# team-ergo-unipi/ergo_uvo

Hardware: AMD Instinct MI355X
Metric: stereo frame-pairs/sec (detect+match+pose) @1920x1080, 3k kpts (higher is better)
Workload: dtype f32+f64

## Files before the change

### ergo_uvo_amd/csrc/surf.hip

```cpp
#include "uvo_ctx.h"
#include <type_traits>
#include <string.h>
#include "uvo_math.h"
#include <algorithm>
#include <utility>
#include <vector>
#include <string>

namespace uvo {

struct ImgPair { const uint8_t* img[2]; int32_t* sum[2]; int32_t* planes[2]; int pw, pstride; int* cand_n; int* big_n; int* surv_n; };
struct AreaTab;
struct CandOut { uvo_keypoint* cand[2]; int* count; int cap; };
struct SurvOut { Survivor* list; int* count; int cap; };
static_assert(sizeof(Survivor) == 128, "a survivor record is 32 words");
struct SortArgs { const uvo_keypoint* cand[2]; const int* cand_n; uvo_keypoint* out[2]; int* out_n[2]; int* rank; int cap;
                  int4* big_par; int* big_n; int* gate_nqa; int gate_min_features; };
struct DescArgs { const uint8_t* img[2]; uvo_keypoint* kps[2]; float* desc[2]; const int* n[2]; const float* DW;
                  const int4* big_par; const int* big_n; const int* big_large; int cap;
                  const AreaTab* tabs; const int* iscale;
                  int extended;
                  const int32_t* sum[2]; const float* ori_w; int* ori_drop; };
struct LaneArgs { ImgPair ip; int32_t* part; SurvOut sv; CandOut out; SortArgs sa; DescArgs da; uint8_t* patch; const int4* big_in; int4* big_out; int* big_large; };
static const int kStripRows = 8;
// ... 1126 lines not shown

__host__ __device__ __forceinline__ AreaTab area_tab(int dx, int ssize, double scale)
{
    AreaTab t;
    double fsx1 = dx * scale;
    double fsx2 = fsx1 + scale;
    double cellWidth = scale < ssize - fsx1 ? scale : ssize - fsx1;
    int sx1 = cv_ceil_d(fsx1), sx2 = cv_floor_d(fsx2);
    sx2 = sx2 < ssize - 1 ? sx2 : ssize - 1;
    sx1 = sx1 < sx2 ? sx1 : sx2;
    t.sx1 = sx1; t.sx2 = sx2;
    t.has_first = sx1 - fsx1 > 1e-3;
    t.a_first = (float)((sx1 - fsx1) / cellWidth);
    t.a_mid = (float)(1.0 / cellWidth);
    t.has_last = fsx2 - sx2 > 1e-3;
    double a = fsx2 - sx2; if (a > 1.) a = 1.; if (a > cellWidth) a = cellWidth;
    t.a_last = (float)(a / cellWidth);
    return t;
}

__device__ __forceinline__ uint8_t sat_u8(float v) { int iv = cv_round_f(v); return (uint8_t)(iv < 0 ? 0 : iv > 255 ? 255 : iv); }


__device__ __forceinline__ void describe_tail(const DescArgs& a, int im, int k, const int (*PATCH)[21])
{
    const int tid = threadIdx.x;
    __shared__ float DX[20][20], DY[20][20];
    __shared__ float vec[128];
    __shared__ float s_scale;
    const int dsize = a.extended ? 128 : 64;
    for (int o = tid; o < 400; o += 256) {
        int i = o / 20, j = o - i * 20;
        float dw = a.DW[o];
        float vx = (PATCH[i][j+1] - PATCH[i][j] + PATCH[i+1][j+1] - PATCH[i+1][j]) * dw;
        float vy = (PATCH[i+1][j] - PATCH[i][j] + PATCH[i+1][j+1] - PATCH[i][j+1]) * dw;
        DX[i][j] = vx; DY[i][j] = vy;
    }
    __syncthreads();
    if (tid < dsize) {
        float acc = 0.f;
        if (!a.extended) {
            int cell = tid >> 2, comp = tid & 3, ci = cell >> 2, cj = cell & 3;
            for (int y = ci * 5; y < ci * 5 + 5; y++)
                for (int x = cj * 5; x < cj * 5 + 5; x++) {
                    float t = (comp & 1) ? DY[y][x] : DX[y][x];
                    acc += (comp & 2) ? (float)fabs(t) : t;
                }
        } else {
            int cell = tid >> 3, comp = tid & 7, ci = cell >> 2, cj = cell & 3;
            for (int y = ci * 5; y < ci * 5 + 5; y++)
                for (int x = cj * 5; x < cj * 5 + 5; x++) {
                    const float tx = DX[y][x], ty = DY[y][x];
                    const float val = comp < 4 ? tx : ty, sel = comp < 4 ? ty : tx;
                    const bool take = (comp & 2) ? sel < 0 : sel >= 0;
                    if (take) acc += (comp & 1) ? (float)fabs(val) : val;
                }
        }
        vec[tid] = acc;
    }
    __syncthreads();
    if (tid == 0) {
        double square_mag = 0;
        for (int kk = 0; kk < dsize; kk++) square_mag += vec[kk] * vec[kk];
        s_scale = (float)(1. / (sqrt(square_mag) + FLT_EPSILON));
    }
    __syncthreads();
    if (tid < dsize) a.desc[im][(size_t)k * dsize + tid] = vec[tid] * s_scale;
}

static const int kTapBatch = 16;
static const int kPatchStride = 448;
__device__ __forceinline__ int sgpr_i(int v) { return __builtin_amdgcn_readfirstlane(v); }
__device__ __forceinline__ int ssel_lt(int a, int b, int x, int y)
{
    int r;
    asm volatile("s_cmp_lt_i32 %1, %2\n\ts_cselect_b32 %0, %3, %4" : "=s"(r) : "s"(a), "s"(b), "s"(x), "s"(y) : "scc");
    return r;
}
__device__ __forceinline__ float sgpr_f(float v) { return __int_as_float(__builtin_amdgcn_readfirstlane(__float_as_int(v))); }

struct ColTask { int y0, n, h1, w; float a_first, a_mid, a_last; };

template <int PX> __device__ __forceinline__ unsigned px_load(ImgRsrc rs, int voff, int soff);
template <> __device__ __forceinline__ unsigned px_load<1>(ImgRsrc rs, int voff, int soff) { return __builtin_amdgcn_raw_buffer_load_b8(rs, voff, soff, 0); }
template <> __device__ __forceinline__ unsigned px_load<2>(ImgRsrc rs, int voff, int soff) { return __builtin_amdgcn_raw_buffer_load_b16(rs, voff, soff, 0); }
template <> __device__ __forceinline__ unsigned px_load<4>(ImgRsrc rs, int voff, int soff) { return __builtin_amdgcn_raw_buffer_load_b32(rs, voff, soff, 0); }

template <int PX, int Q>
struct AreaCol {
    ImgRsrc rs; int w, h1;
    int x[Q], voff[Q];
    float acc[Q][PX];
    __device__ __forceinline__ AreaCol(ImgRsrc rs_, int w_, int h_, int lane, int xa) : rs(rs_), w(w_), h1(h_ - 1)
    {
#pragma unroll
        for (int q = 0; q < Q; q++) { x[q] = xa + PX * (lane + 64 * q); voff[q] = x[q] < w - PX ? x[q] : w - PX; }
    }
    __device__ __forceinline__ void load(const ColTask& t, int tap, unsigned (&v)[Q]) const
    {
        int y = t.y0 - tap; y = y > 0 ? y : 0; y = y < h1 ? y : h1;
        const int soff = y * w;
#pragma unroll
        for (int q = 0; q < Q; q++) v[q] = px_load<PX>(rs, voff[q], soff);
    }
    static __device__ __forceinline__ float px_times(unsigned v, int p, float alpha) { return (float)(int)((v >> (8 * p)) & 255u) * alpha; }
    __device__ __forceinline__ void first(const unsigned (&v)[Q], float alpha)
    {
#pragma unroll
        for (int q = 0; q < Q; q++)
#pragma unroll
            for (int p = 0; p < PX; p++) acc[q][p] = px_times(v[q], p, alpha);
    }
    __device__ __forceinline__ void accum(const unsigned (&v)[Q], float alpha)
    {
#pragma unroll
        for (int q = 0; q < Q; q++)
#pragma unroll
            for (int p = 0; p < PX; p++) acc[q][p] += px_times(v[q], p, alpha);
    }
    template <int N> __device__ __forceinline__ void taps_static(const ColTask& t)
    {
        unsigned v[N][Q];
#pragma unroll
        for (int i = 0; i < N; i++) load(t, i, v[i]);
        first(v[0], t.a_first);
#pragma unroll
        for (int i = 1; i < N - 1; i++) accum(v[i], t.a_mid);
        if (N > 1) accum(v[N - 1], t.a_last);
    }
    __device__ __forceinline__ void taps_any(const ColTask& t)
    {
        constexpr int B = Q == 1 ? 8 : (Q == 2 ? 7 : 4);
        const int last = t.n - 1;
        unsigned v0[Q], vl[Q], v[B][Q];
        load(t, 0, v0);
        load(t, last > 0 ? last : 0, vl);
        first(v0, t.n > 0 ? t.a_first : 0.f);
        for (int tap = 1; tap < last; tap += B) {
#pragma unroll
            for (int i = 0; i < B; i++) load(t, tap + i < last ? tap + i : last, v[i]);
#pragma unroll
            for (int i = 0; i < B; i++) accum(v[i], tap + i < last ? t.a_mid : 0.f);
        }
        accum(vl, last > 0 ? t.a_last : 0.f);
    }
    __device__ __forceinline__ void taps(const ColTask& t)
    {
        if (Q == 1) {
            switch (t.n) {
            case 1: taps_static<1>(t); break;   case 2: taps_static<2>(t); break;   case 3: taps_static<3>(t); break;
            case 4: taps_static<4>(t); break;   case 5: taps_static<5>(t); break;   case 6: taps_static<6>(t); break;
            case 7: taps_static<7>(t); break;   case 8: taps_static<8>(t); break;   case 9: taps_static<9>(t); break;
            case 10: taps_static<10>(t); break; case 11: taps_static<11>(t); break; case 12: taps_static<12>(t); break;
            case 13: taps_static<13>(t); break; case 14: taps_static<14>(t); break;
            default: taps_any(t); break;
            }
        } else if (Q == 2 && PX == 1) {
            switch (t.n) {
            case 1: taps_static<1>(t); break;   case 2: taps_static<2>(t); break;   case 3: taps_static<3>(t); break;
            case 4: taps_static<4>(t); break;   case 5: taps_static<5>(t); break;   case 6: taps_static<6>(t); break;
            case 7: taps_static<7>(t); break;   case 8: taps_static<8>(t); break;
            default: taps_any(t); break;
            }
        } else taps_any(t);
    }
    __device__ __forceinline__ void store(int lane, int start_x, int win_size, float* __restrict__ row) const
    {
        const int xlo = start_x > 0 ? start_x : 0, xhi = start_x + win_size < w ? start_x + win_size : w;
        const int sh = start_x & 3;
        float* dst = row + sh - start_x;
#pragma unroll
        for (int q = 0; q < Q; q++) {
            if (x[q] < xhi) {
                if (PX == 4) *reinterpret_cast<float4*>(dst + x[q]) = make_float4(acc[q][0], acc[q][1], acc[q][2], acc[q][3]);
                else if (PX == 2) *reinterpret_cast<float2*>(dst + x[q]) = make_float2(acc[q][0], acc[q][1]);
                else dst[x[q]] = acc[q][0];
            }
        }
        const int ilo = xlo - start_x, ihi = xhi - start_x;
        if (ilo > 0) { const float b = row[sh + ilo]; for (int i = lane; i < ilo; i += 64) row[sh + i] = b; }
        if (ihi < win_size) { const float b = row[sh + ihi - 1]; for (int i = ihi + lane; i < win_size; i += 64) row[sh + i] = b; }
    }
};

template <int PX, int Q>
__device__ __forceinline__ void area_column(ImgRsrc rs, int lane, int start_x, int win_size, const ColTask& t, float* __restrict__ row)
{
    const int xlo = start_x > 0 ? start_x : 0;
    AreaCol<PX, Q> c(rs, t.w, t.h1 + 1, lane, xlo & ~(PX - 1));
    c.taps(t);
    c.store(lane, start_x, win_size, row);
}
__device__ __forceinline__ ColTask col_task(const AreaTab& ty, int dx, int start_y, int w, int h)
{
    const int sx1 = __builtin_amdgcn_readlane(ty.sx1, dx), sx2 = __builtin_amdgcn_readlane(ty.sx2, dx);
    const float a_first = __int_as_float(__builtin_amdgcn_readlane(__float_as_int(ty.a_first), dx));
    const float a_mid = __int_as_float(__builtin_amdgcn_readlane(__float_as_int(ty.a_mid), dx));
    const float a_last = __int_as_float(__builtin_amdgcn_readlane(__float_as_int(ty.a_last), dx));
    const bool has_first = __builtin_amdgcn_readlane((int)ty.has_first, dx) != 0, has_last = __builtin_amdgcn_readlane((int)ty.has_last, dx) != 0;
    const int c_begin = has_first ? sx1 - 1 : sx1, c_end = has_last ? sx2 + 1 : sx2;
    const int bf = sgpr_i(__float_as_int(a_first)), bm = sgpr_i(__float_as_int(a_mid)), bl = sgpr_i(__float_as_int(a_last));
    ColTask t;
    t.y0 = start_y - c_begin; t.n = c_end - c_begin; t.h1 = h - 1; t.w = w;
    t.a_first = __int_as_float(ssel_lt(c_begin, sx1, bf, ssel_lt(c_begin, sx2, bm, bl)));
    t.a_mid = a_mid;
    t.a_last = __int_as_float(ssel_lt(c_end - 1, sx1, bf, ssel_lt(c_end - 1, sx2, bm, bl)));
    return t;
}

__device__ __forceinline__ void describe_keypoint(const DescArgs& a, int w, int h, int k, int im)
{
    const int tid = threadIdx.x;
    const uvo_keypoint kp = a.kps[im][k];
    const float size = kp.size;
    const float s = size * 1.2f / 9.0f;
    const int win_size = (int)((20 + 1) * s);
    if (win_size > kSmallWin) return;
    extern __shared__ __align__(16) unsigned char smem_desc[];
    float* buf = reinterpret_cast<float*>(smem_desc);
    const int bp = (win_size + 3) | 1;
    __shared__ AreaTab tab[21];
    __shared__ int PATCH[21][21];
    const uint8_t* __restrict__ img = a.img[im];
    const float win_offset = -(float)(win_size - 1) / 2;
    const int start_x = cv_round_f(kp.x + win_offset);
    const int start_y = cv_round_f(kp.y - win_offset);
    const double inv_scale = (double)21 / win_size;
    const double scale = 1. / inv_scale;
    const int iscale = cv_round_d(scale);
    const bool area_fast = fabs(scale - iscale) < DBL_EPSILON;

    if (area_fast) {
        for (int o = tid; o < 441; o += 256) {
            int dy = o / 21, dx = o - dy * 21;
            int sum = 0;
            for (int sx = 0; sx < iscale; sx++) {
                int y = start_y - (dx * iscale + sx); y = y > 0 ? y : 0; y = y < h - 1 ? y : h - 1;
                for (int sy = 0; sy < iscale; sy++) {
                    int x = start_x + dy * iscale + sy; x = x > 0 ? x : 0; x = x < w - 1 ? x : w - 1;
                    sum += img[(size_t)y * w + x];
                }
            }
            int result;
            if (iscale == 2) result = (sum + 2) >> 2;
            else { float sc = 1.f / (iscale * iscale); result = sat_u8(sum * sc); }
            PATCH[dy][dx] = result;
        }
    } else {
        if (tid < 21) tab[tid] = area_tab(tid, win_size, scale);
        __syncthreads();
        {
            const int wv = sgpr_i(tid >> 6), lane = tid & 63;
            const AreaTab ty = tab[lane % 21];
            const int xlo = start_x > 0 ? start_x : 0, xhi = start_x + win_size < w ? start_x + win_size : w;
            const ImgRsrc rs = img_rsrc(img, w * h);
            const int sx = sgpr_i(start_x), sy = sgpr_i(start_y), ws = sgpr_i(win_size);
            if (xhi <= xlo) { for (int it = tid; it < 21 * bp; it += 256) buf[it] = 0.f; }
            else if (xhi - xlo <= 64) {
                AreaCol<1, 1> c(rs, w, h, lane, xlo);
                for (int dx = wv; dx < 21; dx += 4) { const ColTask ct = col_task(ty, dx, sy, w, h); c.taps(ct); c.store(lane, sx, ws, buf + dx * bp); }
            } else {
                AreaCol<1, 2> c(rs, w, h, lane, xlo);
                for (int dx = wv; dx < 21; dx += 4) { const ColTask ct = col_task(ty, dx, sy, w, h); c.taps(ct); c.store(lane, sx, ws, buf + dx * bp); }
            }
        }
        __syncthreads();
        for (int o = tid; o < 441; o += 256) {
            int dy = o / 21, dx = o - dy * 21;
            const AreaTab ty = tab[dy];
            const float* col = buf + dx * bp + (start_x & 3);
            float sum = 0.f;
            if (ty.has_first) sum += ty.a_first * col[ty.sx1 - 1];
            for (int r = ty.sx1; r < ty.sx2; r++) sum += ty.a_mid * col[r];
            if (ty.has_last) sum += ty.a_last * col[ty.sx2];
            PATCH[dy][dx] = sat_u8(sum);
        }
    }
    __syncthreads();
    describe_tail(a, im, k, PATCH);
}

static const int kOriRadius = 6, kOriWin = 60, kOriInc = 5, kOriSamples = 113;
__device__ __forceinline__ float fast_atan2_deg(float y, float x)
{
    const float sc = (float)(180 / 3.14159265358979323846);
    const float p1 = 0.9997878412794807f * sc, p3 = -0.3258083974640975f * sc, p5 = 0.1555786518463281f * sc, p7 = -0.04432655554792128f * sc;
    const float ax = fabsf(x), ay = fabsf(y);
    float a, c, c2;
    if (ax >= ay) { c = ay / (ax + (float)DBL_EPSILON); c2 = c * c; a = (((p7 * c2 + p5) * c2 + p3) * c2 + p1) * c; }
    else { c = ax / (ay + (float)DBL_EPSILON); c2 = c * c; a = 90.f - (((p7 * c2 + p5) * c2 + p3) * c2 + p1) * c; }
    if (x < 0) a = 180.f - a;
    if (y < 0) a = 360.f - a;
    return a;
}
__device__ __forceinline__ void ori_gradients(const int32_t* __restrict__ p, int sw, int gws, float* vx, float* vy)
{
    const float ratio = (float)gws / 4;
    const int c0 = cv_round_f(ratio * 0), c2 = cv_round_f(ratio * 2), c4 = cv_round_f(ratio * 4);
    auto box = [&](int x1, int y1, int x2, int y2) { return p[y1 * sw + x1] + p[y2 * sw + x2] - p[y2 * sw + x1] - p[y1 * sw + x2]; };
    {
        const float w0 = -1 / ((float)(c2 - c0) * (c4 - c0)), w1 = 1 / ((float)(c4 - c2) * (c4 - c0));
        double d = 0;
        d += box(c0, c0, c2, c4) * w0; d += box(c2, c0, c4, c4) * w1;
        *vx = (float)d;
    }
    {
        const float w0 = 1 / ((float)(c4 - c0) * (c2 - c0)), w1 = -1 / ((float)(c4 - c0) * (c4 - c2));
        double d = 0;
        d += box(c0, c0, c4, c2) * w0; d += box(c0, c2, c4, c4) * w1;
        *vy = (float)d;
    }
}

__global__ __launch_bounds__(256) void k_surf_orientation(DescArgs a, int w, int h)
{
    const int im = blockIdx.y, lane = threadIdx.x & 63, wv = threadIdx.x >> 6;
    const int n = *a.n[im];
    const int k = blockIdx.x * 4 + wv;
    __shared__ float sX[4][128], sY[4][128]; __shared__ int sA[4][128];
    if (k >= n) return;
    uvo_keypoint kp = a.kps[im][k];
    const float s = kp.size * 1.2f / 9.0f;
    const int gws = 2 * cv_round_f(2 * s);
    const int sum_rows = h + 1, sw = w + 1;
    const int32_t* __restrict__ sum = a.sum[im];
    int cnt_before = 0;
    for (int pass = 0; pass < 3; pass++) {
        const int cell = pass * 64 + lane;
        bool inside = false, valid = false; float vx = 0, vy = 0;
        if (cell < 169) {
            const int i = cell / 13 - kOriRadius, j = cell % 13 - kOriRadius;
            inside = i * i + j * j <= kOriRadius * kOriRadius;
            if (inside) {
                const int x = cv_round_f(kp.x + i * s - (float)(gws - 1) / 2), y = cv_round_f(kp.y + j * s - (float)(gws - 1) / 2);
                if (!(y < 0 || y >= sum_rows - gws || x < 0 || x >= sw - gws)) {
                    valid = true;
                    ori_gradients(sum + (size_t)y * sw + x, sw, gws, &vx, &vy);
                    const float wgt = a.ori_w[(i + kOriRadius) * 13 + (j + kOriRadius)];
                    vx *= wgt; vy *= wgt;
                }
            }
        }
        const unsigned long long m = __ballot(valid);
        if (valid) {
            const int pos = cnt_before + __popcll(m & ((1ull << lane) - 1ull));
            sX[wv][pos] = vx; sY[wv][pos] = vy; sA[wv][pos] = cv_round_f(fast_atan2_deg(vy, vx));
        }
        cnt_before += __popcll(m);
    }
    const int nangle = cnt_before;
    __builtin_amdgcn_fence(__ATOMIC_ACQ_REL, "wavefront");
    __builtin_amdgcn_wave_barrier();
    if (nangle == 0) { if (lane == 0) atomicAdd(a.ori_drop, 1); return; }
    float best_mod = 0.f, bx = 0.f, by = 0.f; int best_i = 1 << 30;
    for (int d = lane; d < 360 / kOriInc; d += 64) {
        const int i = d * kOriInc;
        float sumx = 0.f, sumy = 0.f;
        for (int j = 0; j < nangle; j++) {
            const int dd = abs(sA[wv][j] - i);
            if (dd < kOriWin / 2 || dd > 360 - kOriWin / 2) { sumx += sX[wv][j]; sumy += sY[wv][j]; }
        }
        const float mod = sumx * sumx + sumy * sumy;
// ... 185 lines not shown
                                        const float alpha = j < tx.sx1 ? tx.a_first : (j < tx.sx2 ? tx.a_mid : tx.a_last);
                                        b += v * alpha;
                                    }
                                    if (j + 1 >= c_end) {
                                        buf[dx][tid] = b; b = 0.f; dx++;
                                        if (dx < 21) tx = tab[dx];
                                        continue;
                                    }
                                    break;
                                }
                            }
                        }
                    }
                } else {
                    for (int e = tid; e < 21 * nr; e += 256) {
                        const int dx = e / nr, il = e - dx * nr;
                        int x = start_x + r0 + il; x = x > 0 ? x : 0; x = x < ncols1 ? x : ncols1;
                        const int c_begin = tap_begin(dx), c_end = tap_end(dx);
                        const AreaTab tx = tab[dx];
                        float b = 0.f;
                        int isum = 0;
                        for (int c0 = c_begin; c0 < c_end; c0 += 8) {
                            int v[8];
#pragma unroll
                            for (int q = 0; q < 8; q++) {
                                int y = start_y - (c0 + q); y = y > 0 ? y : 0; y = y < nrows1 ? y : nrows1;
                                v[q] = img[(size_t)y * w + x];
                            }
#pragma unroll
                            for (int q = 0; q < 8; q++) {
                                const int cc = c0 + q;
                                if (cc >= c_end) continue;
                                if (iscale) isum += v[q];
                                else {
                                    const float alpha = cc < tx.sx1 ? tx.a_first : (cc < tx.sx2 ? tx.a_mid : tx.a_last);
                                    b += v[q] * alpha;
                                }
                            }
                        }
                        if (iscale) reinterpret_cast<int*>(&buf[dx][0])[il] = isum;
                        else buf[dx][il] = b;
                    }
                }
                __syncthreads();
                if (tid < 21) {
                    if (iscale) { for (int r = 0; r < nr; r++) visum += reinterpret_cast<const int*>(&buf[tid][0])[r]; }
                    else for (int r = 0; r < nr; r++) {
                        const int rr = r0 + r;
                        const float beta = rr < ty.sx1 ? ty.a_first : (rr < ty.sx2 ? ty.a_mid : ty.a_last);
                        vsum += beta * buf[tid][r];
                    }
                }
                __syncthreads();
            }
            if (tid < 21) {
                int result;
                if (!iscale) result = sat_u8(vsum);
                else if (iscale == 2) result = (visum + 2) >> 2;
                else { const float sc = 1.f / (iscale * iscale); result = sat_u8(visum * sc); }
                patch[((size_t)im * a.cap + k) * kPatchStride + dy * 21 + tid] = (uint8_t)result;
            }
        }
        __syncthreads();
    }
}
__global__ __launch_bounds__(256) void k_descriptor_wide_finish(DescArgs a, const uint8_t* __restrict__ patch)
{
    const int im = blockIdx.y, tid = threadIdx.x;
    const int n = *a.n[im];
    __shared__ int PATCH[21][21];
    for (int k = blockIdx.x; k < n; k += gridDim.x) {
        const float s = a.kps[im][k].size * 1.2f / 9.0f;
        if ((int)((20 + 1) * s) <= kMaxWin) continue;
        const uint8_t* src = patch + ((size_t)im * a.cap + k) * kPatchStride;
        for (int o = tid; o < 441; o += 256) PATCH[o / 21][o % 21] = src[o];
        __syncthreads();
        describe_tail(a, im, k, PATCH);
        __syncthreads();
    }
}

__device__ __forceinline__ void descriptor64_small(const DescArgs& a, int w, int h, int bx, int nbx, int im)
{
    const int n = *a.n[im];
    for (int k = bx; k < n; k += nbx) {
        describe_keypoint(a, w, h, k, im);
        __syncthreads();
    }
}
static const int kBigRow = 768;
__device__ __forceinline__ void descriptor64_big(const DescArgs& a, int w, int h, uint8_t* __restrict__ patch, int bx, int nbx, int im)
{
    const int lane = threadIdx.x & 63, wv = sgpr_i(threadIdx.x >> 6);
    const int nb = a.big_n[im], nl = min(a.big_large[im], nb);
    extern __shared__ __align__(16) unsigned char smem_desc[];
    float* bufrow0 = reinterpret_cast<float*>(smem_desc) + wv * kBigRow;
    const uint8_t* __restrict__ img = a.img[im];
    const ImgRsrc rs = img_rsrc(img, w * h);
    const int nt1 = nl * 21, ntask = nt1 + (nb - nl) * 7, NW = nbx * 4, wid = bx * 4 + wv;
    auto task_of = [&](int r) { return r * NW + ((r & 1) ? NW - 1 - wid : wid); };
    auto entry_of = [&](int t) { return t < nt1 ? t / 21 : nl + (t - nt1) / 7; };
    const int tl = lane % 21;
    int4 par_next = make_int4(0, 0, 0, 0);
    AreaTab tab_next = a.tabs[tl];
    if (task_of(0) < ntask) { par_next = a.big_par[im * a.cap + entry_of(task_of(0))]; tab_next = a.tabs[min(par_next.y & 0xFFFF, kMaxWin) * 21 + tl]; }
    for (int r = 0; r * NW < ntask; r++) {
        const int t = task_of(r);
        const int4 par = par_next;
        const AreaTab ty = tab_next;
        if (task_of(r + 1) < ntask) {
            par_next = a.big_par[im * a.cap + entry_of(task_of(r + 1))];
            tab_next = a.tabs[min(par_next.y & 0xFFFF, kMaxWin) * 21 + tl];
        }
        if (t >= ntask) continue;
        const int e = entry_of(t);
        const int ncols = t < nt1 ? 1 : 3, dx0 = t < nt1 ? t - e * 21 : 3 * ((t - nt1) - (e - nl) * 7);
        const int bstride = 256;
        const int win_size = sgpr_i(par.y) & 0xFFFF, start_x = sgpr_i(par.z), start_y = sgpr_i(par.w);
        const int iscale = sgpr_i(par.y) >> 16;
        const bool area_fast = iscale != 0;
        uint8_t* out = patch + ((size_t)im * a.cap + e) * kPatchStride;
        const int xlo = start_x > 0 ? start_x : 0, xhi = start_x + win_size < w ? start_x + win_size : w;
        const bool vec_ok = (w & 3) == 0 && xlo < xhi;
        const int xa = xlo & ~3, ilo = xlo - start_x, ihi = xhi - start_x;
        if (area_fast) {
            for (int d = 0; d < ncols; d++) {
                const int dx = dx0 + d;
                int* colsum = reinterpret_cast<int*>(bufrow0 + d * bstride);
                if (vec_ok) {
                    for (int x4 = xa + 4 * lane; x4 < xhi; x4 += 256) {
                        int s0 = 0, s1 = 0, s2 = 0, s3 = 0;
                        for (int sx = 0; sx < iscale; sx++) {
                            int y = start_y - (dx * iscale + sx); y = y > 0 ? y : 0; y = y < h - 1 ? y : h - 1;
                            const unsigned v = *reinterpret_cast<const unsigned*>(img + ((unsigned)(y * w) + (unsigned)x4));
                            s0 += v & 255u; s1 += (v >> 8) & 255u; s2 += (v >> 16) & 255u; s3 += v >> 24;
                        }
                        const int c = x4 - start_x;
                        if (c >= ilo) colsum[c] = s0;
                        if (c + 1 >= ilo && c + 1 < ihi) colsum[c + 1] = s1;
                        if (c + 2 >= ilo && c + 2 < ihi) colsum[c + 2] = s2;
                        if (c + 3 >= ilo && c + 3 < ihi) colsum[c + 3] = s3;
                    }
                    if (ilo > 0) { const int v = colsum[ilo]; for (int c = lane; c < ilo; c += 64) colsum[c] = v; }
                    if (ihi < win_size) { const int v = colsum[ihi - 1]; for (int c = ihi + lane; c < win_size; c += 64) colsum[c] = v; }
                } else
                for (int c = lane; c < win_size; c += 64) {
                    int x = start_x + c; x = x > 0 ? x : 0; x = x < w - 1 ? x : w - 1;
                    int sum = 0;
                    for (int sx = 0; sx < iscale; sx++) {
                        int y = start_y - (dx * iscale + sx); y = y > 0 ? y : 0; y = y < h - 1 ? y : h - 1;
                        sum += img[(size_t)y * w + x];
                    }
                    colsum[c] = sum;
                }
            }
            __builtin_amdgcn_wave_barrier();
            if (lane < 21 * ncols) {
                const int d = lane / 21, dy = lane - d * 21;
                const int* colsum = reinterpret_cast<const int*>(bufrow0 + d * bstride);
                int sum = 0;
                for (int sy = 0; sy < iscale; sy++) sum += colsum[dy * iscale + sy];
                int result;
                if (iscale == 2) result = (sum + 2) >> 2;
                else { float sc = 1.f / (iscale * iscale); result = sat_u8(sum * sc); }
                out[dy * 21 + dx0 + d] = (uint8_t)result;
            }
        } else {
            for (int d = 0; d < ncols; d++) {
                const int dx = dx0 + d;
                float* bufrow = bufrow0 + d * bstride;
                if (vec_ok) {
// ... 259 lines not shown
            c->d_hess_order_cap = (size_t)ngroups;
        }
        UVO_HIP_TRY(c, hipMemcpyAsync(c->d_hess_order, c->h_hess_order.data(), sizeof(uint32_t) * (size_t)ngroups, hipMemcpyHostToDevice, c->stream));
        UVO_HIP_TRY(c, hipStreamSynchronize(c->stream));
        c->hess_order_key[0] = nb0; c->hess_order_key[1] = nb1; c->hess_order_key[2] = nb23;
    }
    return UVO_OK;
}

static uvo_status surf_detect_general(Ctx* c, const LaneArgs& LA, int nimg, float thr)
{
    const int w = c->img_w, h = c->img_h;
    const int no = c->p.SURF_OCTAVES_NUMBER, nl = c->p.SURF_OCTAVES_LAYERS;
    const GenLayer* tab = static_cast<const GenLayer*>(c->d_gen_tab);
    const int gx = std::min(1024, (w * h + 255) / 256);
    {
        StageTimer t(c, ST_HESSIAN_O0);
        hipLaunchKernelGGL(k_scale_space_det, dim3(gx, no * (nl + 2), nimg), dim3(256), 0, c->stream, LA, tab, c->d_gen_planes, c->gen_img_floats, w);
        UVO_HIP_TRY(c, hipGetLastError());
    }
    {
        StageTimer t(c, ST_HESSIAN_O0 + 1);
        hipLaunchKernelGGL(k_scale_space_nms, dim3(gx, no * nl, nimg), dim3(256), 0, c->stream, LA, tab, c->d_gen_planes, c->gen_img_floats, nl, w, h, thr);
        UVO_HIP_TRY(c, hipGetLastError());
    }
    return UVO_OK;
}

static uvo_status surf_detect_tuned(Ctx* c, const LaneArgs& LA, int nimg, float thr)
{
    constexpr int TW0 = kMergedTW0, TH0 = kMergedTH0, TW1 = kMergedTW1, TH1 = kO1TileRows;
    constexpr size_t lds0 = hessian_c_tile_lds<0, TW0, TH0>(), lds1 = hessian_c_tile_lds<1, TW1, TH1>(), lds = lds0 > lds1 ? lds0 : lds1;
    static_assert(lds <= 54600, "three blocks of the merged detection launch must fit a CU's 160 KB of LDS");
    const int w = c->img_w, h = c->img_h;
    const OctavePat* ops = reinterpret_cast<const OctavePat*>(c->h_octpat.data());
    const int total = merged_grid(ops).total;
    if (total > 0) {
        auto kern = k_hessian_nms_all<TW0, TH0>;
        static bool lds_raised[64] = {false};
        UVO_HIP_TRY(c, raise_dynamic_lds(c, kern, lds, lds_raised));
        StageTimer t(c, ST_HESSIAN_O0);
        HessDims hd;
        for (int o = 0; o < 4; o++) {
            OctDims& d = hd.o[o];
            for (int l = 0; l < 5; l++) { d.L[l].samples_i = ops[o].L[l].samples_i; d.L[l].samples_j = ops[o].L[l].samples_j; }
            d.rows = ops[o].rows; d.cols = ops[o].cols; d.octave = ops[o].octave;
            for (int l = 0; l < 3; l++) d.nms_margin[l] = ops[o].nms_margin[l];
        }
        Ctx::TraceRec* trh = (c->trace_on && c->trace_cur >= 0) ? &c->trace[c->trace_cur] : nullptr;
        if (trh) (void)hipEventRecord(trh->ev[6], c->stream);
        hipLaunchKernelGGL(kern, dim3(total, nimg), dim3(kP23Threads), lds, c->stream, LA, w, h, hd, thr, c->d_hess_order);
        if (trh) { (void)hipEventRecord(trh->ev[7], c->stream); trh->det_marked = true; }
        UVO_HIP_TRY(c, hipGetLastError());
    }
    {
        StageTimer t(c, ST_HESSIAN_O0 + c->p.SURF_OCTAVES_NUMBER - 1);
        hipLaunchKernelGGL(k_hessian_finish, dim3((c->surv_cap + kFinishPerWg - 1) / kFinishPerWg), dim3(256), 0, c->stream, LA, static_cast<const OctavePat*>(c->d_octpat), w, h);
        UVO_HIP_TRY(c, hipGetLastError());
    }
    return UVO_OK;
}

static uvo_status surf_order(Ctx* c, const LaneArgs& LA, int nimg)
{
    StageTimer t(c, ST_SORT);
    hipLaunchKernelGGL(k_order, dim3(1, nimg), dim3(kOrderThreads), 0, c->stream, LA, c->d_area_iscale);
    if (c->cap > kOrderCap) {
        const int tiles_max = ((c->cap + 255) / 256) * ((c->cap + kSortChunk - 1) / kSortChunk);
        hipLaunchKernelGGL(k_rank_partial, dim3(tiles_max < 512 ? tiles_max : 512, nimg), dim3(256), 0, c->stream, LA);
        hipLaunchKernelGGL(k_rank_scatter, dim3((c->cap + 255) / 256, nimg), dim3(256), 0, c->stream, LA);
        hipLaunchKernelGGL(k_big_sort, dim3(nimg), dim3(1024), 0, c->stream, LA, c->cap, c->d_area_iscale);
    }
    UVO_HIP_TRY(c, hipGetLastError());
    return UVO_OK;
}

static uvo_status surf_describe(Ctx* c, const LaneArgs& LA, int nimg)
{
    const int w = c->img_w, h = c->img_h;
    StageTimer t(c, ST_DESCRIPTOR);
    const bool wide = c->sh->surf_detection_path == 1 || widest_window(c, w, h) > kMaxWin;
    const int kWideGrid = 128;
    if (c->p.SURF_UPRIGHT) {
        const size_t lds_small = sizeof(float) * 21 * ((kSmallWin + 3) | 1), lds_big = sizeof(float) * 4 * kBigRow;
        const int nbig = 1024;
        const int hint = c->sh->kp_hint;
        int nsmall = hint > 0 ? ((hint + hint / 4 + 255) & ~255) : c->cap;
        nsmall = nsmall < 512 ? 512 : (nsmall > c->cap ? c->cap : nsmall);
        hipLaunchKernelGGL(k_descriptor64, dim3((nbig + nsmall) * nimg), dim3(256), lds_small > lds_big ? lds_small : lds_big, c->stream, DescLane{ { LA } }, w, h, nbig, nimg);
        hipLaunchKernelGGL(k_descriptor64_big_finish, dim3(1024, nimg), dim3(256), 0, c->stream, LA);
        if (wide) {
            hipLaunchKernelGGL(k_descriptor_wide<false>, dim3(21 * kWideGrid, nimg), dim3(256), 0, c->stream, LA.da, w, h, LA.patch);
            hipLaunchKernelGGL(k_descriptor_wide_finish, dim3(kWideGrid, nimg), dim3(256), 0, c->stream, LA.da, LA.patch);
        }
    } else {
        const DescArgs& da = LA.da;
        const size_t lds_rot = sizeof(float) * 21 * (kMaxWin + 1);
        static bool lds_raised[64] = {false};
        UVO_HIP_TRY(c, raise_dynamic_lds(c, k_descriptor_rot, lds_rot, lds_raised));
        hipLaunchKernelGGL(k_surf_orientation, dim3((c->cap + 3) / 4, nimg), dim3(256), 0, c->stream, da, w, h);
        hipLaunchKernelGGL(k_descriptor_rot, dim3(2048, nimg), dim3(256), lds_rot, c->stream, da, w, h);
        if (wide) {
            hipLaunchKernelGGL(k_descriptor_wide<true>, dim3(21 * kWideGrid, nimg), dim3(256), 0, c->stream, da, w, h, LA.patch);
            hipLaunchKernelGGL(k_descriptor_wide_finish, dim3(kWideGrid, nimg), dim3(256), 0, c->stream, da, LA.patch);
        }
    }
    UVO_HIP_TRY(c, hipGetLastError());
    return UVO_OK;
}

uvo_status surf_detect(Ctx* c, int nimg, int gate_min_features)
{
    UVO_TRY(surf_prepare(c, c->img_w, c->img_h));
    const LaneArgs LA = lane_args(c, nimg, gate_min_features);
    const float thr = (float)c->p.SURF_MIN_HESSIAN;
    UVO_TRY(surf_integral_launch(c, LA, nimg));
    UVO_TRY(general_path(c) ? surf_detect_general(c, LA, nimg, thr) : surf_detect_tuned(c, LA, nimg, thr));
    UVO_TRY(surf_order(c, LA, nimg));
    return surf_describe(c, LA, nimg);
}

uvo_status surf_hessian_layer_debug(Ctx* c, int octave, int layer, float* det, float* trace)
{
    const int w = c->img_w, h = c->img_h;
    if (octave < 0 || octave >= kGenMaxOctaves || layer < 0 || layer > c->p.SURF_OCTAVES_LAYERS + 1 || w <= 0) {
        c->err = "hessian_layer: octave 0..7, layer 0..SURF_OCTAVES_LAYERS + 1 of the context's parameters, after an image";
        return UVO_INVALID_ARG;
    }
    GenLayer op;
    make_gen_layer(octave, layer, w, h, &op);
    size_t n = (size_t)op.rows * op.cols;
    if (n == 0) return UVO_OK;
    float *d_det = nullptr, *d_tr = nullptr;
    UVO_HIP_TRY(c, hipMalloc(&d_det, sizeof(float) * n * 2));
    d_tr = d_det + n;
    UVO_HIP_TRY(c, hipMemsetAsync(d_det, 0, sizeof(float) * n * 2, c->stream));
    const LayerPat& lp = op.lp;
    if (lp.samples_i > 0) {
        dim3 g((lp.samples_j + 255) / 256, lp.samples_i);
        hipLaunchKernelGGL(k_hessian_layer_debug, g, dim3(256), 0, c->stream, c->d_sum[0], w, h, lp, op.step, op.rows, op.cols, d_det, d_tr);
    }
    UVO_HIP_TRY(c, hipMemcpyAsync(det, d_det, sizeof(float) * n, hipMemcpyDeviceToHost, c->stream));
    UVO_HIP_TRY(c, hipMemcpyAsync(trace, d_tr, sizeof(float) * n, hipMemcpyDeviceToHost, c->stream));
    UVO_HIP_TRY(c, hipStreamSynchronize(c->stream));
    (void)hipFree(d_det);
    return UVO_OK;
}

}
```

Baseline: 4101.

## Describe small SURF keypoints one per wavefront with direct separable area gathers

Rewrites the small-window upright descriptor so that each 64-lane wavefront handles one keypoint, instead of a whole 256-thread block per keypoint. Per-wave LDS replaces shared block buffers, and wave barriers replace block-wide __syncthreads. The area resampling now gathers each of the 441 patch entries directly, using dword buffer loads with byte alignment and perm-based edge clamping, templated on tap count, rather than a column-buffer pass followed by a row pass. The grid is shrunk 4x and the dynamic LDS for the small path is dropped. It risks numeric differences in summation order and fewer blocks in flight.

```diff
diff --git a/ergo_uvo_amd/csrc/surf.hip b/ergo_uvo_amd/csrc/surf.hip
--- a/ergo_uvo_amd/csrc/surf.hip
+++ b/ergo_uvo_amd/csrc/surf.hip
@@ -1232,8 +1232,6 @@
 struct ColTask { int y0, n, h1, w; float a_first, a_mid, a_last; };
 
 template <int PX> __device__ __forceinline__ unsigned px_load(ImgRsrc rs, int voff, int soff);
-template <> __device__ __forceinline__ unsigned px_load<1>(ImgRsrc rs, int voff, int soff) { return __builtin_amdgcn_raw_buffer_load_b8(rs, voff, soff, 0); }
-template <> __device__ __forceinline__ unsigned px_load<2>(ImgRsrc rs, int voff, int soff) { return __builtin_amdgcn_raw_buffer_load_b16(rs, voff, soff, 0); }
 template <> __device__ __forceinline__ unsigned px_load<4>(ImgRsrc rs, int voff, int soff) { return __builtin_amdgcn_raw_buffer_load_b32(rs, voff, soff, 0); }
 
 template <int PX, int Q>
@@ -1303,13 +1301,6 @@
             case 7: taps_static<7>(t); break;   case 8: taps_static<8>(t); break;   case 9: taps_static<9>(t); break;
             case 10: taps_static<10>(t); break; case 11: taps_static<11>(t); break; case 12: taps_static<12>(t); break;
             case 13: taps_static<13>(t); break; case 14: taps_static<14>(t); break;
-            default: taps_any(t); break;
-            }
-        } else if (Q == 2 && PX == 1) {
-            switch (t.n) {
-            case 1: taps_static<1>(t); break;   case 2: taps_static<2>(t); break;   case 3: taps_static<3>(t); break;
-            case 4: taps_static<4>(t); break;   case 5: taps_static<5>(t); break;   case 6: taps_static<6>(t); break;
-            case 7: taps_static<7>(t); break;   case 8: taps_static<8>(t); break;
             default: taps_any(t); break;
             }
         } else taps_any(t);
@@ -1358,76 +1349,177 @@
     return t;
 }
 
-__device__ __forceinline__ void describe_keypoint(const DescArgs& a, int w, int h, int k, int im)
-{
-    const int tid = threadIdx.x;
+static const int kWaveLds = kPatchStride + 128 * (int)sizeof(float);
+__device__ __forceinline__ void wave_sync() { __builtin_amdgcn_fence(__ATOMIC_ACQ_REL, "wavefront"); __builtin_amdgcn_wave_barrier(); }
+
+struct AreaRun { int begin, n; float wf, wm, wl; };
+static_assert(21 * sizeof(AreaRun) <= 128 * sizeof(float), "a wave keeps its runs where its descriptor vector goes");
+__device__ __forceinline__ AreaRun area_run(const AreaTab& t, bool unit)
+{
+    AreaRun r;
+    const int end = t.has_last ? t.sx2 + 1 : t.sx2;
+    r.begin = t.has_first ? t.sx1 - 1 : t.sx1; r.n = end - r.begin;
+    int bf = __float_as_int(t.a_first), bm = __float_as_int(t.a_mid), bl = __float_as_int(t.a_last);
+    asm volatile("" : "+v"(bf), "+v"(bm), "+v"(bl));
+    r.wf = __int_as_float(r.begin < t.sx1 ? bf : (r.begin < t.sx2 ? bm : bl));
+    r.wl = __int_as_float(end - 1 < t.sx1 ? bf : (end - 1 < t.sx2 ? bm : bl));
+    r.wm = __int_as_float(bm);
+    if (unit) r.wf = r.wm = r.wl = 1.f;
+    return r;
+}
+__device__ __forceinline__ float run_weight(const AreaRun& r, int i) { return i >= r.n ? 0.f : (i == r.n - 1 ? r.wl : (i == 0 ? r.wf : r.wm)); }
+
+template <int NT, bool CLAMP>
+struct RowFetch {
+    int xc, h1; unsigned sel_lo, sel_hi;
+    __device__ __forceinline__ RowFetch(int x0, int w, int h) : xc(x0), h1(h - 1), sel_lo(0), sel_hi(0)
+    {
+        if (CLAMP) {
+            xc = x0 < w - NT ? x0 : w - NT; xc = xc > 0 ? xc : 0;
+#pragma unroll
+            for (int i = 0; i < NT; i++) {
+                int x = x0 + i; x = x > 0 ? x : 0; x = x < w - 1 ? x : w - 1;
+                if (i < 4) sel_lo |= (unsigned)(x - xc) << (8 * i); else sel_hi |= (unsigned)(x - xc) << (8 * (i - 4));
+            }
+        }
+    }
+    __device__ __forceinline__ void load(ImgRsrc rs, int w, int y, unsigned (&d)[3]) const
+    {
+        if (CLAMP) { y = y > 0 ? y : 0; y = y < h1 ? y : h1; }
+        const int oa = (y * w + xc) & ~3;
+        d[0] = __builtin_amdgcn_raw_buffer_load_b32(rs, oa, 0, 0); d[1] = __builtin_amdgcn_raw_buffer_load_b32(rs, oa + 4, 0, 0);
+        d[2] = NT <= 5 ? 0u : __builtin_amdgcn_raw_buffer_load_b32(rs, oa + 8, 0, 0);
+    }
+    __device__ __forceinline__ void bytes(int w, int y, const unsigned (&d)[3], unsigned& lo, unsigned& hi) const
+    {
+        if (CLAMP) { y = y > 0 ? y : 0; y = y < h1 ? y : h1; }
+        const int sh = (y * w + xc) & 3;
+        lo = __builtin_amdgcn_alignbyte(d[1], d[0], sh); hi = __builtin_amdgcn_alignbyte(d[2], d[1], sh);
+        if (CLAMP) { const unsigned l = __builtin_amdgcn_perm(hi, lo, sel_lo), u = __builtin_amdgcn_perm(hi, lo, sel_hi); lo = l; hi = u; }
+    }
+};
+template <int NT, bool CLAMP>
+__device__ __forceinline__ float gather_entry(ImgRsrc rs, int w, int h, int start_x, int start_y, const AreaRun* __restrict__ tab, int dx, int dy)
+{
+    constexpr int B = NT <= 5 ? NT : 4;
+    float H[NT];
+    {
+        const AreaRun c = tab[dx];
+        const RowFetch<NT, CLAMP> f(start_x + tab[dy].begin, w, h);
+        const int y0 = start_y - c.begin;
+#pragma unroll
+        for (int t0 = 0; t0 < NT; t0 += B) {
+            unsigned d[B][3];
+#pragma unroll
+            for (int b = 0; b < B; b++) if (t0 + b < NT) f.load(rs, w, y0 - (t0 + b), d[b]);
+#pragma unroll
+            for (int b = 0; b < B; b++) {
+                const int t = t0 + b;
+                if (t >= NT) continue;
+                unsigned lo, hi;
+                f.bytes(w, y0 - t, d[b], lo, hi);
+                const float alpha = run_weight(c, t);
+#pragma unroll
+                for (int i = 0; i < NT; i++) {
+                    const float p = (float)(int)(((i < 4 ? lo : hi) >> (8 * (i & 3))) & 255u) * alpha;
+                    H[i] = t == 0 ? p : H[i] + p;
+                }
+            }
+        }
+    }
+    const AreaRun r = tab[dy];
+    float sum = 0.f;
+#pragma unroll
+    for (int i = 0; i < NT; i++) sum += run_weight(r, i) * H[i];
+    return sum;
+}
+template <int NT, bool CLAMP>
+__device__ __forceinline__ void gather_patch(ImgRsrc rs, int w, int h, int lane, int start_x, int start_y, const AreaRun* __restrict__ tab, int iscale, float sc, uint8_t* __restrict__ P)
+{
+    for (int j = 0; j < 7; j++) {
+        const int e = lane + 64 * j, ec = e < 441 ? e : 440;
+        const int dx = ec / 21, dy = ec - dx * 21;
+        const float sum = gather_entry<NT, CLAMP>(rs, w, h, start_x, start_y, tab, dx, dy);
+        int result;
+        if (iscale == 0) result = sat_u8(sum);
+        else {
+            const int isum = (int)sum;
+            if (iscale == 2) result = (isum + 2) >> 2;
+            else result = sat_u8(isum * sc);
+        }
+        if (e < 441) P[dy * 21 + dx] = (uint8_t)result;
+    }
+}
+template <bool EXT>
+__device__ __forceinline__ float cell_sum(const uint8_t* __restrict__ P, const float* __restrict__ DW, int d)
+{
+    const int cell = EXT ? d >> 3 : d >> 2, comp = EXT ? d & 7 : d & 3, ci = cell >> 2, cj = cell & 3;
+    float acc = 0.f;
+#pragma unroll 1
+    for (int yy = 0; yy < 5; yy++)
+#pragma unroll
+        for (int xx = 0; xx < 5; xx++) {
+            const int i = ci * 5 + yy, j = cj * 5 + xx;
+            const int p00 = P[i * 21 + j], p01 = P[i * 21 + j + 1], p10 = P[i * 21 + 21 + j], p11 = P[i * 21 + 21 + j + 1];
+            const float dw = DW[i * 20 + j];
+            const float tx = (p01 - p00 + p11 - p10) * dw;
+            const float ty = (p10 - p00 + p11 - p01) * dw;
+            if (!EXT) {
+                const float t = (comp & 1) ? ty : tx;
+                acc += (comp & 2) ? (float)fabs(t) : t;
+            } else {
+                const float val = comp < 4 ? tx : ty, sel = comp < 4 ? ty : tx;
+                const bool take = (comp & 2) ? sel < 0 : sel >= 0;
+                if (take) acc += (comp & 1) ? (float)fabs(val) : val;
+            }
+        }
+    return acc;
+}
+__device__ __forceinline__ void describe_keypoint(const DescArgs& a, ImgRsrc rs, int w, int h, int k, int im, int lane, unsigned char* __restrict__ lds)
+{
     const uvo_keypoint kp = a.kps[im][k];
     const float size = kp.size;
     const float s = size * 1.2f / 9.0f;
     const int win_size = (int)((20 + 1) * s);
     if (win_size > kSmallWin) return;
-    extern __shared__ __align__(16) unsigned char smem_desc[];
-    float* buf = reinterpret_cast<float*>(smem_desc);
-    const int bp = (win_size + 3) | 1;
-    __shared__ AreaTab tab[21];
-    __shared__ int PATCH[21][21];
-    const uint8_t* __restrict__ img = a.img[im];
+    uint8_t* P = lds;
+    float* vec = reinterpret_cast<float*>(lds + kPatchStride);
     const float win_offset = -(float)(win_size - 1) / 2;
-    const int start_x = cv_round_f(kp.x + win_offset);
-    const int start_y = cv_round_f(kp.y - win_offset);
-    const double inv_scale = (double)21 / win_size;
-    const double scale = 1. / inv_scale;
-    const int iscale = cv_round_d(scale);
-    const bool area_fast = fabs(scale - iscale) < DBL_EPSILON;
-
-    if (area_fast) {
-        for (int o = tid; o < 441; o += 256) {
-            int dy = o / 21, dx = o - dy * 21;
-            int sum = 0;
-            for (int sx = 0; sx < iscale; sx++) {
-                int y = start_y - (dx * iscale + sx); y = y > 0 ? y : 0; y = y < h - 1 ? y : h - 1;
-                for (int sy = 0; sy < iscale; sy++) {
-                    int x = start_x + dy * iscale + sy; x = x > 0 ? x : 0; x = x < w - 1 ? x : w - 1;
-                    sum += img[(size_t)y * w + x];
-                }
-            }
-            int result;
-            if (iscale == 2) result = (sum + 2) >> 2;
-            else { float sc = 1.f / (iscale * iscale); result = sat_u8(sum * sc); }
-            PATCH[dy][dx] = result;
+    const int start_x = sgpr_i(cv_round_f(kp.x + win_offset));
+    const int start_y = sgpr_i(cv_round_f(kp.y - win_offset));
+    const int ws = sgpr_i(win_size > 0 ? win_size : 0);
+    const int iscale = sgpr_i(a.iscale[ws]);
+    AreaRun* tab = reinterpret_cast<AreaRun*>(vec);
+    int el = lane; asm volatile("" : "+v"(el));
+    if (el < 21) tab[el] = area_run(a.tabs[ws * 21 + el], iscale != 0);
+    wave_sync();
+    const float sc = sgpr_f(1.f / (iscale * iscale));
+    const int nt = (ws + 20) / 21 + 1;
+    const bool inside = start_x >= 0 && start_x + ws <= w && start_y <= h - 1 && start_y - (ws - 1) >= 0;
+    if (inside) {
+        switch (nt) {
+        case 4: gather_patch<4, false>(rs, w, h, lane, start_x, start_y, tab, iscale, sc, P); break;
+        case 5: gather_patch<5, false>(rs, w, h, lane, start_x, start_y, tab, iscale, sc, P); break;
+        case 6: gather_patch<6, false>(rs, w, h, lane, start_x, start_y, tab, iscale, sc, P); break;
+        case 7: gather_patch<7, false>(rs, w, h, lane, start_x, start_y, tab, iscale, sc, P); break;
+        case 8: gather_patch<8, false>(rs, w, h, lane, start_x, start_y, tab, iscale, sc, P); break;
+        default: gather_patch<3, false>(rs, w, h, lane, start_x, start_y, tab, iscale, sc, P); break;
         }
     } else {
-        if (tid < 21) tab[tid] = area_tab(tid, win_size, scale);
-        __syncthreads();
-        {
-            const int wv = sgpr_i(tid >> 6), lane = tid & 63;
-            const AreaTab ty = tab[lane % 21];
-            const int xlo = start_x > 0 ? start_x : 0, xhi = start_x + win_size < w ? start_x + win_size : w;
-            const ImgRsrc rs = img_rsrc(img, w * h);
-            const int sx = sgpr_i(start_x), sy = sgpr_i(start_y), ws = sgpr_i(win_size);
-            if (xhi <= xlo) { for (int it = tid; it < 21 * bp; it += 256) buf[it] = 0.f; }
-            else if (xhi - xlo <= 64) {
-                AreaCol<1, 1> c(rs, w, h, lane, xlo);
-                for (int dx = wv; dx < 21; dx += 4) { const ColTask ct = col_task(ty, dx, sy, w, h); c.taps(ct); c.store(lane, sx, ws, buf + dx * bp); }
-            } else {
-                AreaCol<1, 2> c(rs, w, h, lane, xlo);
-                for (int dx = wv; dx < 21; dx += 4) { const ColTask ct = col_task(ty, dx, sy, w, h); c.taps(ct); c.store(lane, sx, ws, buf + dx * bp); }
-            }
-        }
-        __syncthreads();
-        for (int o = tid; o < 441; o += 256) {
-            int dy = o / 21, dx = o - dy * 21;
-            const AreaTab ty = tab[dy];
-            const float* col = buf + dx * bp + (start_x & 3);
-            float sum = 0.f;
-            if (ty.has_first) sum += ty.a_first * col[ty.sx1 - 1];
-            for (int r = ty.sx1; r < ty.sx2; r++) sum += ty.a_mid * col[r];
-            if (ty.has_last) sum += ty.a_last * col[ty.sx2];
-            PATCH[dy][dx] = sat_u8(sum);
-        }
-    }
-    __syncthreads();
-    describe_tail(a, im, k, PATCH);
+        if (nt <= 5) gather_patch<5, true>(rs, w, h, lane, start_x, start_y, tab, iscale, sc, P);
+        else gather_patch<8, true>(rs, w, h, lane, start_x, start_y, tab, iscale, sc, P);
+    }
+    wave_sync();
+    const int dsize = a.extended ? 128 : 64;
+    int tl = lane; asm volatile("" : "+v"(tl));
+    if (!a.extended) vec[tl] = cell_sum<false>(P, a.DW, tl);
+    else for (int d = tl; d < 128; d += 64) vec[d] = cell_sum<true>(P, a.DW, d);
+    wave_sync();
+    double square_mag = 0;
+    for (int kk = 0; kk < dsize; kk++) square_mag += vec[kk] * vec[kk];
+    const float scale = (float)(1. / (sqrt(square_mag) + FLT_EPSILON));
+    for (int d = tl; d < dsize; d += 64) a.desc[im][(size_t)k * dsize + d] = vec[d] * scale;
+    wave_sync();
 }
 
 static const int kOriRadius = 6, kOriWin = 60, kOriInc = 5, kOriSamples = 113;
@@ -1779,11 +1871,11 @@
 
 __device__ __forceinline__ void descriptor64_small(const DescArgs& a, int w, int h, int bx, int nbx, int im)
 {
+    __shared__ __align__(16) unsigned char s_wave[4][kWaveLds];
+    const int lane = threadIdx.x & 63, wv = sgpr_i(threadIdx.x >> 6);
     const int n = *a.n[im];
-    for (int k = bx; k < n; k += nbx) {
-        describe_keypoint(a, w, h, k, im);
-        __syncthreads();
-    }
+    const ImgRsrc rs = img_rsrc(a.img[im], (w * h + 3) & ~3);
+    for (int k = 4 * bx + wv; k < n; k += 4 * nbx) describe_keypoint(a, rs, w, h, k, im, lane, s_wave[wv]);
 }
 static const int kBigRow = 768;
 __device__ __forceinline__ void descriptor64_big(const DescArgs& a, int w, int h, uint8_t* __restrict__ patch, int bx, int nbx, int im)
@@ -2209,12 +2301,13 @@
     const bool wide = c->sh->surf_detection_path == 1 || widest_window(c, w, h) > kMaxWin;
     const int kWideGrid = 128;
     if (c->p.SURF_UPRIGHT) {
-        const size_t lds_small = sizeof(float) * 21 * ((kSmallWin + 3) | 1), lds_big = sizeof(float) * 4 * kBigRow;
+        const size_t lds_big = sizeof(float) * 4 * kBigRow;
         const int nbig = 1024;
         const int hint = c->sh->kp_hint;
         int nsmall = hint > 0 ? ((hint + hint / 4 + 255) & ~255) : c->cap;
         nsmall = nsmall < 512 ? 512 : (nsmall > c->cap ? c->cap : nsmall);
-        hipLaunchKernelGGL(k_descriptor64, dim3((nbig + nsmall) * nimg), dim3(256), lds_small > lds_big ? lds_small : lds_big, c->stream, DescLane{ { LA } }, w, h, nbig, nimg);
+        nsmall = (nsmall + 3) / 4;
+        hipLaunchKernelGGL(k_descriptor64, dim3((nbig + nsmall) * nimg), dim3(256), lds_big, c->stream, DescLane{ { LA } }, w, h, nbig, nimg);
         hipLaunchKernelGGL(k_descriptor64_big_finish, dim3(1024, nimg), dim3(256), 0, c->stream, LA);
         if (wide) {
             hipLaunchKernelGGL(k_descriptor_wide<false>, dim3(21 * kWideGrid, nimg), dim3(256), 0, c->stream, LA.da, w, h, LA.patch);
```

After: 4232, median of 6. 1.03x the previous value.
